# mheinz757/AgglomerationMultigrid1D

Hardware: NVIDIA B200
Metric: FP64 V-cycle DOF-updates/s (higher is better)
Workload: dtype f64

## Files before the change

### agglomerationmultigrid1d_b200/csrc/amg1d.cu

```cuda
#include <cuda_runtime.h>

#include <algorithm>
#include <cmath>
#include <cstdarg>
#include <cstdio>
#include <cstring>
#include <string>
#include <vector>

#ifdef AMG1D_WITH_NCCL
#include <dlfcn.h>
#include <nccl.h>
#endif

#include "../../include/amg1d.h"
#include "kernels_generic.cuh"
#include "kernels_fused.cuh"
#include "kernels_multi.cuh"
#include "kernels_rows.cuh"
#include "direct_bcr.cuh"
#include "device_setup.cuh"
#include "halo_p2p.cuh"

#define AMG1D_VERSION 100
#define PAD_FRONT 64
#define PAD_BACK 64
#define MULTI_SLOTS 8
static_assert(MULTI_MAX_COLS == AMG1D_MAX_COLS, "kernels_multi.cuh and amg1d.h disagree on the column limit");

namespace {

std::string g_create_error;

struct DVec {
    double* raw = nullptr;
    double* p = nullptr;
    int64_t len = 0;
    bool in_arena = false;
};

struct DevBuf {
    double* p = nullptr;
    ~DevBuf() { if (p) cudaFree(p); }
    cudaError_t alloc(int64_t doubles) { return cudaMalloc((void**)&p, (size_t)(doubles > 0 ? doubles : 1) * 8); }
    DevBuf() = default;
    DevBuf(const DevBuf&) = delete;
    DevBuf& operator=(const DevBuf&) = delete;
};

struct Level {
    bool set = false;
    int64_t n = 0;
    int64_t n_glob = 0;
    int64_t start = 0;
    int gl = 0, gr = 0;
    bool sharded = false;
    bool present = true;
    bool proxy = false;
    double* mat_alloc = nullptr;
    int m = 0;
    int diag = 0;
    int K = 0;
    MatDesc md = {};
    int64_t base_n = 0;
    double* flux[9] = {nullptr, nullptr, nullptr, nullptr, nullptr, nullptr, nullptr, nullptr, nullptr};
    bool smooth_tri = false;
    int dv_rec = 0;
    double* smat_alloc = nullptr;
    double* smat = nullptr;
    MatDesc smd = {};
    int64_t n_host = 0;
    double* mat = nullptr;
    int64_t* perm = nullptr;
    std::vector<double> h_lo, h_di, h_up;
    int64_t mat_bytes = 0;
    double* pat = nullptr;
    int pat_head = 0, pat_tail = 0;
    std::vector<double> pat_host;
};

struct Transfer {
    bool set = false;
    int64_t n_fine = 0, n_coarse = 0;
    int mf = 0, mc = 0;
    int64_t* parent = nullptr;
    int64_t* cp = nullptr;
    std::vector<int64_t> h_parent;
    int ratio = 1, shift = 0, base = 0, period = 0, n_head = 0, n_tail = 0;
    double* P0 = nullptr;
    double* P1 = nullptr;
    int64_t nblk = 0;
    bool single_parent_uniform = false;
    bool closed = false;
    bool fusable = false;
    int64_t p_first = 0;
    int reach = 0;
    int64_t cover_extra = 0;
};

struct Column {
    struct Vecs { DVec x[2], b; int cur = 0; };
    std::vector<Vecs> lv;
    double* scal = nullptr;
    double* partial = nullptr;
    struct { DVec x, p, ap; } cg;
};

struct GraphEntry {
    cudaGraphExec_t exec = nullptr;
    int pre = -1, post = -1, norm = -1, zero0 = -1;
    double alpha = 0.0;
    unsigned mask = 0;
    int64_t launches = 0;
    uint64_t stamp = 0;
};

}

struct amg1d {
    int device = 0;
    cudaStream_t stream = nullptr;
    bool own_stream = false;
    int n_levels = 0;
    std::vector<Level> L;
    std::vector<Transfer> T;
    bool finalized = false;
    std::string err;
    DVec scratch;
    double* stage = nullptr;
    int64_t stage_len = 0;
    int64_t partial_cap = 0;
    Column res;
    bool norm_valid = false;
    bool dev_problem = true;
    double* h_scal = nullptr;
    double* coarse_fac = nullptr;
    int opt_fused = 1, opt_graph = 1;
    int64_t opt_coarse_cta = 1024;
    int opt_compress = 1;
    int opt_pdl = 1;
    int opt_rows = 64;
    int opt_rows_rpt = 0;
    int opt_dvrec = 4;
    int opt_dvrec_max = 4;
    int opt_dvreg = 0;
    int opt_pipe = 1;
    int64_t opt_pipe_min = 500000;
    int opt_pattern = 0;
    int tail_start = -1;
    TailLevel* d_tail = nullptr;
    TailPlan tail_plan_ = {};
    std::vector<TailLevel> tail_host;
    uint64_t tail_gen = 0;
    GraphEntry graphs[4];
    uint64_t graph_clock = 0;
    int64_t launches_per_cycle = 0;
    BcrSolver coarse_bcr;
    std::vector<BcrSolver> direct;
    int64_t launch_counter = 0;
    int64_t device_bytes = 0;
    int opt_profile = 0;
    struct Prof { std::vector<cudaEvent_t> ev; };
    std::vector<Prof> prof;
    int rank = 0, nranks = 1;
    int ghost_depth = 4;
    int64_t shard_min = 8192;
    int gather_level = -1;
#ifdef AMG1D_WITH_NCCL
    ncclComm_t comm = nullptr;
#endif
// ... 109 lines not shown
}

int column_alloc(amg1d* h, Column& col, bool cg) {
    const bool levels = col.lv.empty();
    int rc = AMG1D_OK;
    if (levels) {
        col.lv.resize((size_t)h->n_levels);
        for (int l = 0; l < h->n_levels && rc == AMG1D_OK; ++l) {
            const Level& lv = h->L[l];
            Column::Vecs& v = col.lv[(size_t)l];
            if (!lv.present && !lv.proxy) continue;
            const bool arena = lv.sharded && h->p2p.arena;
            for (DVec* d : {&v.x[0], &v.b, &v.x[1]})
                if (rc == AMG1D_OK && (d != &v.x[1] || lv.present))
                    rc = arena ? vec_from_arena(h, *d, lv.n, lv.m) : vec_alloc(h, *d, lv.n, lv.m);
        }
        if (rc == AMG1D_OK) rc = dev_alloc(h, (void**)&col.partial, (h->partial_cap + 256) * 8);
    }
    if (rc == AMG1D_OK && cg && !col.cg.x.raw)
        for (DVec* d : {&col.cg.x, &col.cg.p, &col.cg.ap})
            if (rc == AMG1D_OK) rc = vec_alloc(h, *d, h->L[0].n, h->L[0].m);
    if (rc != AMG1D_OK) {
        if (levels) column_free(h, col);
        else { vec_release(h, col.cg.x); vec_release(h, col.cg.p); vec_release(h, col.cg.ap); }
        cudaGetLastError();
    }
    return rc;
}

inline dim3 gblock(int m) {
    int z = 256 / (AMG1D_TILE * m);
    if (z < 1) z = 1;
    return dim3(AMG1D_TILE, m, z);
}
inline unsigned ggrid(int64_t n, int m) {
    const int z = gblock(m).z;
    return (unsigned)((amg1d_tiles(n) + z - 1) / z);
}

#define LAUNCH_CHECK() CK(cudaGetLastError())

bool valid_level(amg1d* h, int l) { return h && l >= 0 && l < h->n_levels; }

TransferMap make_map(const Transfer& t) {
    TransferMap tm;
    tm.parent = t.parent;
    tm.cp = t.cp;
    tm.n_fine = t.n_fine;
    tm.n_coarse = t.n_coarse;
    tm.ratio = t.ratio;
    tm.shift = t.shift;
    tm.base = t.base;
    tm.period = t.period;
    tm.n_head = t.n_head;
    tm.n_tail = t.n_tail;
    return tm;
}

TransferMap make_map_closed(const Transfer& t) {
    TransferMap tm = make_map(t);
    tm.parent = nullptr;
    tm.cp = nullptr;
    return tm;
}

inline const double* tp0(const Transfer& t) { return t.P0 ? t.P0 - t.p_first * (int64_t)(t.mf * t.mc) : nullptr; }
inline const double* tp1(const Transfer& t) { return t.P1 ? t.P1 - t.p_first * (int64_t)(t.mf * t.mc) : nullptr; }

inline int64_t slab_start(int64_t n_glob, int nranks, int r) { return (n_glob / nranks) * r; }
inline int64_t slab_size(int64_t n_glob, int nranks, int r) {
    return n_glob / nranks + (r == nranks - 1 ? n_glob % nranks : 0);
}

#ifdef AMG1D_WITH_NCCL
struct NcclApi {
    void* lib = nullptr;
    decltype(&ncclGetUniqueId) GetUniqueId = nullptr;
    decltype(&ncclCommInitRank) CommInitRank = nullptr;
    decltype(&ncclCommDestroy) CommDestroy = nullptr;
    decltype(&ncclSend) Send = nullptr;
    decltype(&ncclRecv) Recv = nullptr;
    decltype(&ncclAllReduce) AllReduce = nullptr;
    decltype(&ncclAllGather) AllGather = nullptr;
    decltype(&ncclGroupStart) GroupStart = nullptr;
    decltype(&ncclGroupEnd) GroupEnd = nullptr;
    decltype(&ncclGetErrorString) GetErrorString = nullptr;
};
NcclApi g_nccl;

const char* load_nccl() {
    if (g_nccl.lib) return nullptr;
    const char* env = getenv("AMG1D_NCCL_LIB");
    void* lib = env ? dlopen(env, RTLD_NOW | RTLD_LOCAL) : nullptr;
    if (!lib) lib = dlopen("libnccl.so.2", RTLD_NOW | RTLD_LOCAL);
    if (!lib) lib = dlopen("libnccl.so", RTLD_NOW | RTLD_LOCAL);
    if (!lib) return "cannot dlopen libnccl.so.2";
#define NSYM(field, name)                                                    \
    g_nccl.field = reinterpret_cast<decltype(g_nccl.field)>(dlsym(lib, name)); \
    if (!g_nccl.field) return "libnccl lacks " name;
    NSYM(GetUniqueId, "ncclGetUniqueId") NSYM(CommInitRank, "ncclCommInitRank")
    NSYM(CommDestroy, "ncclCommDestroy") NSYM(Send, "ncclSend") NSYM(Recv, "ncclRecv")
    NSYM(AllReduce, "ncclAllReduce") NSYM(AllGather, "ncclAllGather") NSYM(GroupStart, "ncclGroupStart") NSYM(GroupEnd, "ncclGroupEnd")
    NSYM(GetErrorString, "ncclGetErrorString")
#undef NSYM
    g_nccl.lib = lib;
    return nullptr;
}
#endif

int rows_rpt(const amg1d* h, int l) {
    if (h->opt_rows_rpt) return h->opt_rows_rpt;
    return h->opt_pattern && h->L[l].pat ? 3 : 1;
}

int leg_rec(const amg1d* h, const Level& lv, int mc = 0) {
    int rec = (h->opt_dvrec > 0 && lv.dv_rec && lv.m >= h->opt_dvrec && lv.m <= h->opt_dvrec_max)
                  ? (lv.dv_rec | (h->opt_dvreg ? 8 : 0) | ((h->opt_pipe && lv.n >= h->opt_pipe_min) ? 16 : 0)) : 0;
    if (!rec && h->opt_dvrec > 0 && h->opt_dvreg >= 2 && lv.dv_rec && lv.m == 2 && fused_has_dv(lv.m, mc, lv.md.st, lv.diag))
        rec = lv.dv_rec | 8;
    if (h->opt_dvrec > 0 && h->opt_pipe >= 2 && lv.n >= h->opt_pipe_min && lv.dv_rec && lv.m == 2 &&
        fused_has_pp(lv.m, mc, lv.md.st, lv.diag))
        rec = (rec & 8) | lv.dv_rec | 16;
    return rec;
}

PatOp make_pat(const amg1d* h, int l) {
    const Level& lv = h->L[l];
    PatOp po;
    po.tab = h->opt_pattern ? lv.pat : nullptr;
    po.n_glob = lv.n_glob;
    po.n_head = lv.pat_head;
    po.n_tail = lv.pat_tail;
    po.host_interior = (h->opt_pattern == 2 && lv.pat && !lv.pat_host.empty())
                           ? lv.pat_host.data() + (size_t)lv.pat_head * lv.K : nullptr;
    return po;
}

Slab make_slab(amg1d* h, int l) {
    Slab sl;
    const Level& lv = h->L[l];
    sl.gl = lv.gl;
    sl.gr = lv.gr;
    sl.e_off = lv.start;
    sl.c_off = 0;
    sl.nc = 0;
    if (l + 1 < h->n_levels) {
        const Level& lc = h->L[l + 1];
        sl.c_off = lv.sharded ? slab_start(lc.n_glob, h->nranks, h->rank) : 0;
        sl.nc = lv.sharded ? slab_size(lc.n_glob, h->nranks, h->rank) : lc.n_glob;
    }
    return sl;
}

#ifdef AMG1D_WITH_NCCL
#define NCK(call)                                                                              \
    do {                                                                                       \
        ncclResult_t r_ = (call);                                                              \
        if (r_ != ncclSuccess)                                                                 \
            return fail(h, AMG1D_ERR_NCCL, "%s failed: %s (%s:%d)", #call, g_nccl.GetErrorString(r_), \
                        __FILE__, __LINE__);                                                   \
    } while (0)

int op_halo(amg1d* h, double* v, int64_t n, int m, double* v2 = nullptr, int64_t n2 = 0, int m2 = 0) {
    NCK(g_nccl.GroupStart());
    for (int k = 0; k < 2; ++k) {
        double* p = k == 0 ? v : v2;
        if (!p) continue;
        const int64_t nn = k == 0 ? n : n2;
        const int mm = k == 0 ? m : m2;
        const int64_t cnt = (int64_t)h->ghost_depth * mm;
        if (h->rank > 0) {
            NCK(g_nccl.Send(p, cnt, ncclDouble, h->rank - 1, h->comm, h->stream));
            NCK(g_nccl.Recv(p - cnt, cnt, ncclDouble, h->rank - 1, h->comm, h->stream));
        }
        if (h->rank < h->nranks - 1) {
            NCK(g_nccl.Send(p + (nn - h->ghost_depth) * mm, cnt, ncclDouble, h->rank + 1, h->comm, h->stream));
            NCK(g_nccl.Recv(p + nn * mm, cnt, ncclDouble, h->rank + 1, h->comm, h->stream));
        }
    }
    NCK(g_nccl.GroupEnd());
    h->launch_counter++;
    return AMG1D_OK;
}

int op_gather_rhs(amg1d* h, Column& col, int g) {
    Level& lg = h->L[g];
    double* b = col.lv[(size_t)g].b.p;
    NCK(g_nccl.GroupStart());
    if (h->rank == 0) {
        for (int r = 1; r < h->nranks; ++r)
            NCK(g_nccl.Recv(b + slab_start(lg.n_glob, h->nranks, r) * lg.m,
                            slab_size(lg.n_glob, h->nranks, r) * lg.m, ncclDouble, r, h->comm, h->stream));
    } else {
        NCK(g_nccl.Send(b, slab_size(lg.n_glob, h->nranks, h->rank) * lg.m, ncclDouble, 0, h->comm,
                        h->stream));
    }
    NCK(g_nccl.GroupEnd());
    h->launch_counter++;
    return AMG1D_OK;
}

int op_scatter_sol(amg1d* h, Column& col, int g) {
    Level& lg = h->L[g];
    Column::Vecs& v = col.lv[(size_t)g];
    const int gd = h->ghost_depth;
    NCK(g_nccl.GroupStart());
    if (h->rank == 0) {
        const double* x = v.x[v.cur].p;
        for (int r = 1; r < h->nranks; ++r) {
            const int64_t e0 = slab_start(lg.n_glob, h->nranks, r) - gd;
            const int64_t e1 = slab_start(lg.n_glob, h->nranks, r) + slab_size(lg.n_glob, h->nranks, r) +
                               (r < h->nranks - 1 ? gd : 0);
            NCK(g_nccl.Send(x + e0 * lg.m, (e1 - e0) * lg.m, ncclDouble, r, h->comm, h->stream));
        }
    } else {
        const int64_t cnt = (slab_size(lg.n_glob, h->nranks, h->rank) + gd +
                             (h->rank < h->nranks - 1 ? gd : 0)) * lg.m;
        NCK(g_nccl.Recv(v.x[0].p - (int64_t)gd * lg.m, cnt, ncclDouble, 0, h->comm, h->stream));
    }
    NCK(g_nccl.GroupEnd());
    h->launch_counter++;
    return AMG1D_OK;
}

__global__ void k_sqrt_inplace(double* v, int slot) { v[slot] = sqrt(v[slot]); }
int op_allreduce_max(amg1d* h, double* dptr, int count) {
    NCK(g_nccl.AllReduce(dptr, dptr, (size_t)count, ncclDouble, ncclMax, h->comm, h->stream));
    return AMG1D_OK;
}
int op_allreduce_norm(amg1d* h, Column& col, int slot, bool take_sqrt) {
    NCK(g_nccl.AllReduce(col.scal + slot, col.scal + slot, 1, ncclDouble, ncclSum, h->comm, h->stream));
    h->launch_counter++;
    if (!take_sqrt) return AMG1D_OK;
    k_sqrt_inplace<<<1, 1, 0, h->stream>>>(col.scal, slot);
    h->launch_counter++;
    LAUNCH_CHECK();
    return AMG1D_OK;
}

#define AMG1D_P2P_MAXL 48
struct P2PXchg {
    cudaIpcMemHandle_t hnd;
    int32_t ok, n_sharded;
    int64_t off[AMG1D_P2P_MAXL][3];
    int64_t n[AMG1D_P2P_MAXL];
};

int nccl_allgather_host(amg1d* h, const void* mine, void* all, size_t bytes) {
    DevBuf snd, rcv;
    CK(snd.alloc((int64_t)(bytes + 7) / 8));
    CK(rcv.alloc((int64_t)(bytes * h->nranks + 7) / 8));
    CK(cudaMemcpyAsync(snd.p, mine, bytes, cudaMemcpyHostToDevice, h->stream));
    NCK(g_nccl.AllGather(snd.p, rcv.p, bytes, ncclChar, h->comm, h->stream));
    CK(cudaMemcpyAsync(all, rcv.p, bytes * h->nranks, cudaMemcpyDeviceToHost, h->stream));
    CK(cudaStreamSynchronize(h->stream));
    return AMG1D_OK;
}

int p2p_alloc_arena(amg1d* h) {
    amg1d::P2P& P = h->p2p;
    int n_sh = 0;
    int64_t total = 0;
    for (int l = 0; l < h->n_levels; ++l) {
        const Level& lv = h->L[l];
        if (!lv.sharded) continue;
        ++n_sh;
        total += 3 * arena_round((PAD_FRONT + lv.n * lv.m + PAD_BACK) * 8);
    }
    if (n_sh == 0 || n_sh > AMG1D_P2P_MAXL) return AMG1D_OK;
    P.n_ch = 2 * n_sh;
    const int64_t flag_bytes = arena_round((int64_t)2 * P.n_ch * 8);
    total += flag_bytes;
    if (cudaMalloc((void**)&P.arena, (size_t)total) != cudaSuccess) { cudaGetLastError(); P.arena = nullptr; return AMG1D_OK; }
    CK(cudaMemsetAsync(P.arena, 0, (size_t)total, h->stream));
    h->device_bytes += total;
    P.bytes = total;
    P.used = flag_bytes;
    P.flags = reinterpret_cast<unsigned long long*>(P.arena);
    return AMG1D_OK;
}

void p2p_close(amg1d* h) {
    amg1d::P2P& P = h->p2p;
    for (int s = 0; s < 2; ++s)
        if (P.peer[s]) { cudaIpcCloseMemHandle(P.peer[s]); P.peer[s] = nullptr; }
    P.on = false;
}

int p2p_connect(amg1d* h, Column& col) {
    amg1d::P2P& P = h->p2p;
    if (!P.arena) return AMG1D_OK;
    P2PXchg mine;
    memset(&mine, 0, sizeof mine);
    mine.ok = cudaIpcGetMemHandle(&mine.hnd, P.arena) == cudaSuccess ? 1 : 0;
    if (!mine.ok) cudaGetLastError();
    for (int l = 0; l < h->n_levels && l < AMG1D_P2P_MAXL; ++l) {
        const Level& lv = h->L[l];
        if (!lv.sharded) continue;
        ++mine.n_sharded;
        const Column::Vecs& cv = col.lv[(size_t)l];
        const DVec* v[3] = {&cv.x[0], &cv.x[1], &cv.b};
        for (int k = 0; k < 3; ++k) {
            if (!v[k]->in_arena) mine.ok = 0;
            mine.off[l][k] = reinterpret_cast<const char*>(v[k]->p) - P.arena;
        }
        mine.n[l] = lv.n;
// ... 163 lines not shown
            lv.smat, lv.smd, h->scratch.p, zero_guess ? nullptr : xin, xout, lv.n, alpha);
        h->launch_counter++;
        LAUNCH_CHECK();
        return AMG1D_OK;
    }
    if (h->opt_fused && fused_sweep(lv.md, lv.mat, b, xin, xout, lv.n, alpha, zero_guess, h->stream)) {
        h->launch_counter++;
        LAUNCH_CHECK();
        return AMG1D_OK;
    }
    const dim3 blk = gblock(lv.m);
    const size_t sm = (size_t)blk.z * lv.m * AMG1D_TILE * sizeof(double);
    g_sweep<<<ggrid(lv.n, lv.m), blk, sm, h->stream>>>(lv.mat, lv.md, b, xin, xout, lv.n, alpha,
                                                        zero_guess);
    h->launch_counter++;
    LAUNCH_CHECK();
    return AMG1D_OK;
}

int op_apply(amg1d* h, int l, const double* b, const double* x, double* out, int mode) {
    Level& lv = h->L[l];
    g_apply<<<ggrid(lv.n, lv.m), gblock(lv.m), 0, h->stream>>>(lv.mat, lv.md, b, x, out, lv.n, mode);
    h->launch_counter++;
    LAUNCH_CHECK();
    return AMG1D_OK;
}

int op_restrict(amg1d* h, int l, const double* rf, double* rc) {
    Transfer& t = h->T[l];
    const int64_t total = t.n_coarse * t.mc;
    g_restrict<<<(unsigned)((total + 255) / 256), 256, 0, h->stream>>>(make_map(t), t.mf, t.mc, t.P0,
                                                                       t.P1, rf, rc);
    h->launch_counter++;
    LAUNCH_CHECK();
    return AMG1D_OK;
}

int op_prolong(amg1d* h, int l, const double* xc, double* xf, int add) {
    Transfer& t = h->T[l];
    const int64_t total = t.n_fine * t.mf;
    g_prolong<<<(unsigned)((total + 255) / 256), 256, 0, h->stream>>>(make_map(t), t.mf, t.mc, t.P0,
                                                                      t.P1, xc, xf, add);
    h->launch_counter++;
    LAUNCH_CHECK();
    return AMG1D_OK;
}

int op_coarse(amg1d* h, const double* b, double* x) {
    Level& lv = h->L[h->n_levels - 1];
    if (h->coarse_bcr.ready()) {
        CK(h->coarse_bcr.solve(b, x, h->stream, &h->launch_counter));
        return AMG1D_OK;
    }
    g_coarse_solve<<<1, 32, 2 * lv.m * sizeof(double), h->stream>>>(h->coarse_fac, lv.m, lv.n, b, x);
    h->launch_counter++;
    LAUNCH_CHECK();
    return AMG1D_OK;
}

int op_norm(amg1d* h, Column& col, const double* a, const double* c, int64_t n, int slot) {
    int nb = (int)std::min<int64_t>(AMG1D_RED_BLOCKS, (n + AMG1D_RED_THREADS - 1) / AMG1D_RED_THREADS);
    if (nb < 1) nb = 1;
    k_sqdiff_partial<<<nb, AMG1D_RED_THREADS, 0, h->stream>>>(a, c, n, col.partial);
    k_reduce_final<<<1, AMG1D_RED_THREADS, 0, h->stream>>>(col.partial, nb, col.scal, slot,
                                                           h->nranks > 1 ? 0 : 1);
    h->launch_counter += 2;
    LAUNCH_CHECK();
    if (h->nranks > 1) RET(op_allreduce_norm(h, col, slot, true));
    return AMG1D_OK;
}

int op_reduce_partials(amg1d* h, Column& col, int64_t np, int slot, bool take_sqrt) {
    const double* src = col.partial;
    if (np > 8192) {
        double* stage2 = col.partial + h->partial_cap;
        k_sum_partial<<<256, AMG1D_RED_THREADS, 0, h->stream>>>(col.partial, np, stage2);
        h->launch_counter++;
        src = stage2;
        np = 256;
    }
    k_reduce_final<<<1, AMG1D_RED_THREADS, 0, h->stream>>>(src, (int)np, col.scal, slot,
                                                           take_sqrt && h->nranks == 1 ? 1 : 0);
    h->launch_counter++;
    LAUNCH_CHECK();
    if (h->nranks > 1) RET(op_allreduce_norm(h, col, slot, take_sqrt));
    return AMG1D_OK;
}

int op_resnorm(amg1d* h, Column& col, int l, int slot) {
    Level& lv = h->L[l];
    Column::Vecs& v = col.lv[(size_t)l];
    if (lv.sharded) RET(op_halo(h, v.x[v.cur].p, lv.n, lv.m));
    if (h->opt_fused) {
        int nb = 0;
        if (fused_resnorm(lv.md, lv.mat, v.b.p, v.x[v.cur].p, lv.n, col.partial, h->partial_cap, &nb,
                          h->stream)) {
            h->launch_counter++;
            LAUNCH_CHECK();
            return op_reduce_partials(h, col, nb, slot, true);
        }
    }
    RET(op_apply(h, l, v.b.p, v.x[v.cur].p, h->scratch.p, 1));
    return op_norm(h, col, h->scratch.p, nullptr, lv.n * lv.m, slot);
}

int op_dot(amg1d* h, Column& col, const double* a, const double* c, int64_t n, int slot) {
    int nb = (int)std::min<int64_t>(AMG1D_RED_BLOCKS, (n + AMG1D_RED_THREADS - 1) / AMG1D_RED_THREADS);
    if (nb < 1) nb = 1;
    k_dot_partial<<<nb, AMG1D_RED_THREADS, 0, h->stream>>>(a, c, n, col.partial);
    h->launch_counter++;
    LAUNCH_CHECK();
    return op_reduce_partials(h, col, nb, slot, false);
}

int op_matvec_dot(amg1d* h, Column& col, int l, double* x, double* y, int slot) {
    Level& lv = h->L[l];
    if (lv.sharded) RET(op_halo(h, x, lv.n, lv.m));
    int nb = 0;
    if (h->opt_fused && fused_matvec_dot(lv.md, lv.mat, x, y, lv.n, slot >= 0 ? col.partial : nullptr,
                                         h->partial_cap, &nb, h->stream)) {
        h->launch_counter++;
        LAUNCH_CHECK();
        return slot >= 0 ? op_reduce_partials(h, col, nb, slot, false) : AMG1D_OK;
    }
    RET(op_apply(h, l, nullptr, x, y, 0));
    return slot >= 0 ? op_dot(h, col, x, y, lv.n * lv.m, slot) : AMG1D_OK;
}

int prof_mark(amg1d* h, int level, int leg) {
    if (!h->opt_profile) return AMG1D_OK;
    if (h->prof.size() < (size_t)h->n_levels * 2) h->prof.resize((size_t)h->n_levels * 2);
    cudaEvent_t ev;
    CK(cudaEventCreate(&ev));
    CK(cudaEventRecord(ev, h->stream));
    h->prof[level * 2 + leg].ev.push_back(ev);
    return AMG1D_OK;
}

int leg_down(amg1d* h, Column& col, int l, int nPre, double alpha, bool zero0) {
    Level& lv = h->L[l];
    Transfer& t = h->T[l];
    Level& lc = h->L[l + 1];
    Column::Vecs& v = col.lv[(size_t)l];
    Column::Vecs& vc = col.lv[(size_t)l + 1];
    const bool zero = l > 0 || zero0;
    if (zero) v.cur = 0;
    RET(prof_mark(h, l, 0));
    if (lv.sharded && !zero && !h->p2p.on) RET(op_halo(h, v.x[v.cur].p, lv.n, lv.m));
    if (h->opt_fused && t.fusable && !lv.smooth_tri) {
        const int ob = zero ? 0 : 1 - v.cur;
        cudaError_t le = cudaSuccess;
        const bool p2p = h->p2p.on && lv.sharded;
        const HaloLeg hl = p2p ? make_halo_leg(h, l, true, ob) : HaloLeg();
        int fr = fused_down(lv.md, t.mc, make_map_closed(t), nPre, zero, lv.mat, make_pat(h, l), v.b.p, v.x[v.cur].p,
                            v.x[ob].p, tp0(t), tp1(t), vc.b.p, lv.n, lv.n + (lv.gr ? t.cover_extra : 0),
                            alpha, make_slab(h, l), h->stream, h->opt_pdl != 0, &le, leg_rec(h, lv, t.mc), hl);
        if (fr == FUSED_NA && h->opt_rows) {
            if (p2p) RET(op_p2p_wait_for(h, hl));
            fr = rows_down(lv.md, t.mc, make_map_closed(t), nPre, zero, lv.mat, make_pat(h, l), v.b.p, v.x[v.cur].p,
                           v.x[ob].p, tp0(t), tp1(t), vc.b.p, lv.n, lv.n + (lv.gr ? t.cover_extra : 0), alpha,
                           make_slab(h, l), h->opt_rows, rows_rpt(h, l), h->stream, h->opt_pdl != 0, &le);
            if (fr == FUSED_OK && p2p) {
                if (lc.sharded) RET(op_p2p_push(h, col, 2 * l, l, ob, l + 1, 2));
                else RET(op_p2p_push(h, col, 2 * l, l, ob));
            }
        }
        if (fr == FUSED_ERR) return fail(h, AMG1D_ERR_CUDA, "f_down launch failed on level %d: %s", l, cudaGetErrorString(le));
        if (fr == FUSED_OK) {
            v.cur = ob;
            h->launch_counter++;
            LAUNCH_CHECK();
            RET(prof_mark(h, l, 0));
            return AMG1D_OK;
        }
    }
    if (lv.sharded)
        return fail(h, AMG1D_ERR_UNSUPPORTED, "level %d: sharded levels need the fused kernels "
                    "(a block size / transfer with a fused leg, closed-form transfer, option fused = 1)", l);
    if (zero && nPre == 0) CK(cudaMemsetAsync(v.x[0].p, 0, (size_t)v.x[0].len * 8, h->stream));
    for (int s = 0; s < nPre; ++s) {
        if (zero && s == 0) {
            RET(op_sweep(h, l, v.b.p, v.x[0].p, v.x[0].p, alpha, 1));
        } else {
            RET(op_sweep(h, l, v.b.p, v.x[v.cur].p, v.x[1 - v.cur].p, alpha, 0));
            v.cur = 1 - v.cur;
        }
    }
    if (h->opt_fused && t.single_parent_uniform &&
        fused_residual_restrict(lv.md, t.mc, make_map_closed(t), lv.mat, v.b.p, v.x[v.cur].p, t.P0,
                                vc.b.p, lv.n, h->stream)) {
        h->launch_counter++;
        LAUNCH_CHECK();
    } else {
        RET(op_apply(h, l, v.b.p, v.x[v.cur].p, h->scratch.p, 1));
        RET(op_restrict(h, l, h->scratch.p, vc.b.p));
    }
    return prof_mark(h, l, 0);
}

int leg_up(amg1d* h, Column& col, int l, int nPost, double alpha, bool fuse_norm, bool* norm_done, bool* halo_pushed) {
    *halo_pushed = false;
    Level& lv = h->L[l];
    Transfer& t = h->T[l];
    Column::Vecs& v = col.lv[(size_t)l];
    Column::Vecs& vc = col.lv[(size_t)l + 1];
    RET(prof_mark(h, l, 1));
    if (h->opt_fused && t.fusable && !lv.smooth_tri) {
        int nb = 0;
        cudaError_t le = cudaSuccess;
        const bool p2p = h->p2p.on && lv.sharded;
        const int ob = 1 - v.cur;
        const bool push_inside = l > 0 || ob == 0;
        const HaloLeg hl = p2p ? make_halo_leg(h, l, false, push_inside ? ob : -1) : HaloLeg();
        int fr = fused_up(lv.md, t.mc, make_map_closed(t), nPost, lv.mat, make_pat(h, l), v.b.p, v.x[v.cur].p,
                          v.x[1 - v.cur].p, tp0(t), tp1(t), vc.x[vc.cur].p, lv.n, alpha,
                          fuse_norm ? col.partial : nullptr, h->partial_cap, &nb, make_slab(h, l),
                          h->stream, h->opt_pdl != 0, &le, leg_rec(h, lv, t.mc), hl);
        if (fr == FUSED_OK && p2p && push_inside) *halo_pushed = true;
        if (fr == FUSED_NA && h->opt_rows) {
            if (p2p) RET(op_p2p_wait_for(h, hl));
            fr = rows_up(lv.md, t.mc, make_map_closed(t), nPost, lv.mat, make_pat(h, l), v.b.p, v.x[v.cur].p,
                         v.x[1 - v.cur].p, tp0(t), tp1(t), vc.x[vc.cur].p, lv.n, alpha,
                         fuse_norm ? col.partial : nullptr, h->partial_cap, &nb, make_slab(h, l), h->opt_rows,
                         rows_rpt(h, l), h->stream, h->opt_pdl != 0, &le);
        }
        if (fr == FUSED_ERR) return fail(h, AMG1D_ERR_CUDA, "f_up launch failed on level %d: %s", l, cudaGetErrorString(le));
        if (fr == FUSED_OK) {
            v.cur = 1 - v.cur;
            h->launch_counter++;
            LAUNCH_CHECK();
            RET(prof_mark(h, l, 1));
            if (fuse_norm) {
                RET(op_reduce_partials(h, col, nb, 0, true));
                *norm_done = true;
            }
            return AMG1D_OK;
        }
    }
    if (lv.sharded)
        return fail(h, AMG1D_ERR_UNSUPPORTED, "level %d: sharded levels need the fused kernels", l);
    RET(op_prolong(h, l, vc.x[vc.cur].p, v.x[v.cur].p, 1));
    for (int s = 0; s < nPost; ++s) {
        RET(op_sweep(h, l, v.b.p, v.x[v.cur].p, v.x[1 - v.cur].p, alpha, 0));
        v.cur = 1 - v.cur;
    }
    return prof_mark(h, l, 1);
}

int enqueue_vcycle(amg1d* h, Column& col, int nPre, int nPost, double alpha, bool want_norm, bool zero0) {
    const int nl = h->n_levels;
    const int g = h->gather_level;
    bool norm_done = false;
    if (g >= 0) {
        int need = std::max(nPre, nPost) + 1;
        for (int l = 0; l < nl - 1; ++l)
            if (h->L[l].sharded) need = std::max(need, std::max(nPre, nPost) + 1 + h->T[l].reach);
        if (need > h->ghost_depth)
            return fail(h, AMG1D_ERR_ARG, "nPre / nPost need ghost_depth >= %d (option \"ghost_depth\", "
                        "before the first level is set)", need);
    }
    const int ts = (h->tail_start > 0 && h->L[h->tail_start].present) ? h->tail_start : nl;
    const bool p2p = g >= 0 && h->p2p.on;
    bool u0_pushed = false;
    if (p2p) RET(op_p2p_begin_cycle(h));
    for (int l = 0; l < nl - 1 && l < ts; ++l) {
        Level& lv = h->L[l];
        if (!lv.present) break;
        RET(leg_down(h, col, l, nPre, alpha, zero0));
        if (lv.sharded) {
            Level& lc = h->L[l + 1];
            Column::Vecs& v = col.lv[(size_t)l];
            if (p2p) {
                if (!lc.sharded) RET(op_gather_rhs(h, col, l + 1));
            } else if (lc.sharded) RET(op_halo(h, v.x[v.cur].p, lv.n, lv.m, col.lv[(size_t)l + 1].b.p, lc.n, lc.m));
            else {
                RET(op_halo(h, v.x[v.cur].p, lv.n, lv.m));
                RET(op_gather_rhs(h, col, l + 1));
            }
        }
    }
    if (ts < nl) {
        for (int l = ts; l < nl; ++l) col.lv[(size_t)l].cur = 0;
        cudaError_t te = tail_launch(h->L[ts].m, h->d_tail, nl - ts, h->coarse_fac, nPre, nPost, alpha,
                                     h->tail_plan_, h->stream, h->opt_pdl != 0);
        if (te != cudaSuccess) return fail(h, AMG1D_ERR_CUDA, "f_tail launch failed: %s", cudaGetErrorString(te));
        h->launch_counter++;
    } else if (h->L[nl - 1].present) {
        Column::Vecs& v = col.lv[(size_t)nl - 1];
        if (nl > 1 || zero0) v.cur = 0;
        RET(op_coarse(h, v.b.p, v.x[v.cur].p));
    }
    for (int l = std::min(nl - 2, ts - 1); l >= 0; --l) {
        Level& lv = h->L[l];
        Level& lc = h->L[l + 1];
        Column::Vecs& v = col.lv[(size_t)l];
        if (!lv.present) continue;
        if (lv.sharded && !lc.sharded) RET(op_scatter_sol(h, col, l + 1));
        bool pushed = false;
        RET(leg_up(h, col, l, nPost, alpha, want_norm && l == 0, &norm_done, &pushed));
        if (p2p && lv.sharded) {
            if (l == 0) u0_pushed = pushed;
            else if (!pushed) RET(op_p2p_push(h, col, 2 * l + 1, l, v.cur));
        } else if (lv.sharded && l > 0) RET(op_halo(h, v.x[v.cur].p, lv.n, lv.m));
    }
    Column::Vecs& v0 = col.lv[0];
    if (v0.cur != 0) {
        CK(cudaMemcpyAsync(v0.x[0].p, v0.x[1].p, (size_t)v0.x[0].len * 8, cudaMemcpyDeviceToDevice,
                           h->stream));
        v0.cur = 0;
    }
    if (p2p && h->L[0].sharded && !u0_pushed) RET(op_p2p_push(h, col, 1, 0, 0));
    if (want_norm && !norm_done) RET(op_resnorm(h, col, 0, 0));
    return AMG1D_OK;
}

template <class Enqueue>
int replay_vcycle(amg1d* h, GraphEntry (&cache)[4], const GraphEntry& key, bool parity0, int64_t* launches,
                  Enqueue enqueue) {
    if (!h->opt_graph || h->opt_profile) {
        const int64_t c0 = h->launch_counter;
        RET(enqueue());
        *launches = h->launch_counter - c0;
        return AMG1D_OK;
    }
    GraphEntry* ge = nullptr;
    for (auto& g : cache)
        if (g.exec && g.mask == key.mask && g.pre == key.pre && g.post == key.post && g.alpha == key.alpha &&
            g.norm == key.norm && g.zero0 == key.zero0)
            ge = &g;
    if (!ge) {
        ge = &cache[0];
        for (auto& g : cache) if (!g.exec) { ge = &g; break; } else if (g.stamp < ge->stamp) ge = &g;
        if (ge->exec) { cudaGraphExecDestroy(ge->exec); ge->exec = nullptr; }
        if (!parity0) return fail(h, AMG1D_ERR_STATE, "internal: level-0 buffer parity");
        cudaGraph_t g = nullptr;
        const int64_t c0 = h->launch_counter;
        CK(cudaStreamBeginCapture(h->stream, cudaStreamCaptureModeThreadLocal));
        int rc = enqueue();
        cudaError_t ce = cudaStreamEndCapture(h->stream, &g);
        if (rc != AMG1D_OK) { if (g) cudaGraphDestroy(g); return rc; }
        if (ce != cudaSuccess) return fail(h, AMG1D_ERR_CUDA, "graph capture failed: %s", cudaGetErrorString(ce));
        const int64_t n = h->launch_counter - c0;
        h->launch_counter = c0;
        cudaGraphExec_t exec = nullptr;
        ce = cudaGraphInstantiate(&exec, g, 0);
        cudaGraphDestroy(g);
        if (ce != cudaSuccess) return fail(h, AMG1D_ERR_CUDA, "graph instantiate failed: %s", cudaGetErrorString(ce));
        *ge = key;
        ge->exec = exec;
        ge->launches = n;
    }
    ge->stamp = ++h->graph_clock;
    CK(cudaGraphLaunch(ge->exec, h->stream));
    *launches = ge->launches;
    h->launch_counter += ge->launches;
    return AMG1D_OK;
}

int run_vcycle(amg1d* h, Column& col, int nPre, int nPost, double alpha, bool want_norm, bool zero0 = false) {
    if (nPre < 0 || nPost < 0) return fail(h, AMG1D_ERR_ARG, "nPre and nPost must be >= 0");
    GraphEntry key;
    key.pre = nPre; key.post = nPost; key.alpha = alpha; key.norm = (int)want_norm; key.zero0 = (int)zero0; key.mask = 1;
    RET(replay_vcycle(h, h->graphs, key, col.lv[0].cur == 0, &h->launches_per_cycle,
                      [&] { return enqueue_vcycle(h, col, nPre, nPost, alpha, want_norm, zero0); }));
    h->norm_valid = want_norm;
    return AMG1D_OK;
}
// ... 2076 lines not shown
    if (h->nranks > 1) return fail(h, AMG1D_ERR_UNSUPPORTED, "per-level host operations are single-GPU only");
    if (level < 0 || level >= h->n_levels - 1) return fail(h, AMG1D_ERR_ARG, "transfer %d out of range", level);
    if (!xf || !xc) return fail(h, AMG1D_ERR_ARG, "null vector");
    invalidate_graph(h);
    Column::Vecs& vc = h->res.lv[(size_t)level + 1];
    double* cin = vc.x[1 - vc.cur].p;
    RET(to_device(h, level + 1, xc, cin));
    RET(op_prolong(h, level, cin, h->scratch.p, 0));
    return to_host(h, level, h->scratch.p, xf);
}

int amg1d_coarse_solve(amg1d_t* h, double* x, const double* b) {
    RET(check_ready(h));
    if (h->nranks > 1) return fail(h, AMG1D_ERR_UNSUPPORTED, "per-level host operations are single-GPU only");
    if (!x || !b) return fail(h, AMG1D_ERR_ARG, "null vector");
    invalidate_graph(h);
    const int l = h->n_levels - 1;
    Column::Vecs& v = h->res.lv[(size_t)l];
    double* bin = v.x[1 - v.cur].p;
    RET(to_device(h, l, b, bin));
    RET(op_coarse(h, bin, h->scratch.p));
    return to_host(h, l, h->scratch.p, x);
}

int amg1d_direct_solve(amg1d_t* h, int level, double* x, const double* b) {
    RET(check_ready(h));
    if (h->nranks > 1) return fail(h, AMG1D_ERR_UNSUPPORTED, "per-level host operations are single-GPU only");
    if (!valid_level(h, level)) return fail(h, AMG1D_ERR_ARG, "level %d out of range", level);
    if (!x || !b) return fail(h, AMG1D_ERR_ARG, "null vector");
    if (h->direct.size() < (size_t)h->n_levels) h->direct.resize((size_t)h->n_levels);
    BcrSolver& S = h->direct[(size_t)level];
    if (!S.ready()) RET(bcr_factor(h, S, level));
    invalidate_graph(h);
    Column::Vecs& v = h->res.lv[(size_t)level];
    double* bin = v.x[1 - v.cur].p;
    RET(to_device(h, level, b, bin));
    CK(S.solve(bin, h->scratch.p, h->stream, &h->launch_counter));
    return to_host(h, level, h->scratch.p, x);
}

int amg1d_set_option(amg1d_t* h, const char* key, int64_t value) {
    if (!h || !key) return AMG1D_ERR_ARG;
    invalidate_graph(h);
    if (!strcmp(key, "fused")) h->opt_fused = (int)value;
    else if (!strcmp(key, "graph")) h->opt_graph = (int)value;
    else if (!strcmp(key, "pdl")) h->opt_pdl = (int)value;
    else if (!strcmp(key, "rows_window")) {
        if (value != 0 && !rows_window_ok((int)value)) return fail(h, AMG1D_ERR_ARG, "rows_window must be 0, 32 or 64");
        h->opt_rows = (int)value;
    }
    else if (!strcmp(key, "pattern_resident")) {
        if (value < 0 || value > 2) return fail(h, AMG1D_ERR_ARG, "pattern_resident must be 0, 1 or 2");
        h->opt_pattern = (int)value;
    }
    else if (!strcmp(key, "p2p_halo")) {
        if (h->finalized) return fail(h, AMG1D_ERR_STATE, "'p2p_halo' must be set before amg1d_finalize");
        h->opt_p2p = value != 0;
    }
    else if (!strcmp(key, "dinv_registers")) h->opt_dvreg = (int)value;
    else if (!strcmp(key, "leg_pipeline_min")) {
        if (value < 0) return fail(h, AMG1D_ERR_ARG, "leg_pipeline_min must be >= 0");
        h->opt_pipe_min = value;
    }
    else if (!strcmp(key, "recompute_dinv_max")) {
        if (value < 1 || value > 5) return fail(h, AMG1D_ERR_ARG, "recompute_dinv_max must be in [1, 5]");
        h->opt_dvrec_max = (int)value;
    }
    else if (!strcmp(key, "leg_pipeline")) {
        if (value < 0 || value > 2) return fail(h, AMG1D_ERR_ARG, "leg_pipeline must be 0, 1 or 2");
        h->opt_pipe = (int)value;
    }
    else if (!strcmp(key, "recompute_dinv")) {
        if (value < 0) return fail(h, AMG1D_ERR_ARG, "recompute_dinv must be >= 0");
        h->opt_dvrec = (int)value;
    }
    else if (!strcmp(key, "rows_per_thread")) {
        if (value != 0 && !rows_rpt_ok((int)value)) return fail(h, AMG1D_ERR_ARG, "rows_per_thread must be 0 (auto), 1, 2 or 3");
        h->opt_rows_rpt = (int)value;
    }
    else if (!strcmp(key, "coarse_cta_elems")) {
        h->opt_coarse_cta = value;
        if (h->finalized) { CK(cudaSetDevice(h->device)); CK(cudaStreamSynchronize(h->stream)); RET(build_tail(h)); }
    }
    else if (!strcmp(key, "ghost_depth") || !strcmp(key, "shard_min") || !strcmp(key, "compress")) {
        for (auto& lv : h->L)
            if (lv.set) return fail(h, AMG1D_ERR_STATE, "'%s' must be set before the first level", key);
        if (!strcmp(key, "compress")) { h->opt_compress = value != 0; return AMG1D_OK; }
        if (value < 1) return fail(h, AMG1D_ERR_ARG, "'%s' must be >= 1", key);
        if (!strcmp(key, "ghost_depth")) {
            if ((value + 2) * 8 > PAD_FRONT) return fail(h, AMG1D_ERR_ARG, "ghost_depth must be <= %d", PAD_FRONT / 8 - 2);
            h->ghost_depth = (int)value;
        } else h->shard_min = value;
    }
    else if (!strcmp(key, "profile")) {
        h->opt_profile = (int)value;
        for (auto& pr : h->prof) { for (auto ev : pr.ev) cudaEventDestroy(ev); pr.ev.clear(); }
    }
    else return fail(h, AMG1D_ERR_ARG, "unknown option '%s'", key);
    return AMG1D_OK;
}

int64_t amg1d_get_info(amg1d_t* h, const char* key) {
    if (!h || !key) return -1;
    if (!strcmp(key, "kernel_launches")) return h->launch_counter;
    if (!strcmp(key, "launches_per_cycle")) return h->launches_per_cycle;
    if (!strcmp(key, "device_bytes")) return h->device_bytes;
    if (!strcmp(key, "n_levels")) return h->n_levels;
    if (!strcmp(key, "local_elements")) return h->L[0].n;
    if (!strcmp(key, "local_dofs")) return h->L[0].n * h->L[0].m;
    if (!strcmp(key, "local_offset_dofs")) return h->L[0].start * h->L[0].m;
    if (!strcmp(key, "gather_level")) return h->gather_level;
    if (!strcmp(key, "tail_start")) return h->tail_start;
    if (!strcmp(key, "ghost_depth")) return h->ghost_depth;
    if (!strcmp(key, "rows_window")) return h->opt_rows;
    if (!strcmp(key, "rows_per_thread")) return h->opt_rows_rpt;
    if (!strcmp(key, "pattern_resident")) return h->opt_pattern;
    if (!strncmp(key, "pattern:", 8)) {
        const int l = atoi(key + 8);
        return valid_level(h, l) && h->L[l].pat ? 1 : 0;
    }
    if (!strcmp(key, "recompute_dinv")) return h->opt_dvrec;
    if (!strcmp(key, "dinv_registers")) return h->opt_dvreg;
    if (!strcmp(key, "leg_pipeline")) return h->opt_pipe;
    if (!strcmp(key, "leg_pipeline_min")) return h->opt_pipe_min;
    if (!strncmp(key, "leg_pipeline:", 13)) {
        const int l = atoi(key + 13);
        if (!valid_level(h, l) || !h->L[l].set || l + 1 >= h->n_levels || !h->T[l].fusable) return 0;
        if (h->opt_pattern && h->L[l].pat) return 0;
        const int rec = leg_rec(h, h->L[l], h->T[l].mc);
        return ((rec & 16) && (rec & 3) && fused_has_pp(h->L[l].m, h->T[l].mc, h->L[l].md.st, h->L[l].diag)) ? 1 : 0;
    }
    if (!strcmp(key, "p2p_halo")) return h->p2p.on ? 1 : 0;
    if (!strcmp(key, "halo_bytes_per_cycle")) {
        int64_t bytes = 0;
        const int sides = (h->rank > 0) + (h->rank < h->nranks - 1);
        for (int l = 0; l < h->n_levels; ++l) {
            if (!h->L[l].sharded) continue;
            bytes += 2LL * h->ghost_depth * h->L[l].m * 8 * sides;
            if (l + 1 < h->n_levels && h->L[l + 1].sharded) bytes += (int64_t)h->ghost_depth * h->L[l + 1].m * 8 * sides;
        }
        return bytes;
    }
    if (!strcmp(key, "sharded_levels")) {
        int c = 0;
        for (const auto& lv : h->L) c += lv.sharded ? 1 : 0;
        return c;
    }
    if (!strncmp(key, "dinv_pivots:", 12)) {
        const int l = atoi(key + 12);
        return valid_level(h, l) && h->L[l].set ? (h->L[l].dv_rec == 1) : -1;
    }
    if (!strncmp(key, "dinv_recompute:", 15)) {
        const int l = atoi(key + 15);
        if (!valid_level(h, l) || !h->L[l].set || l + 1 >= h->n_levels || !(leg_rec(h, h->L[l], h->T[l].mc) & 3)) return 0;
        if (h->opt_pattern && h->L[l].pat) return 0;
        return (h->L[l].m <= 5 && h->T[l].fusable) ? 1 : 0;
    }
    if (!strncmp(key, "structure:", 10)) {
        const int l = atoi(key + 10);
        return valid_level(h, l) && h->L[l].set ? h->L[l].md.st : -1;
    }
    if (!strncmp(key, "tile_rows:", 10)) {
        const int l = atoi(key + 10);
        return valid_level(h, l) && h->L[l].set ? h->L[l].md.K : -1;
    }
    if (!strcmp(key, "rank")) return h->rank;
    if (!strcmp(key, "nranks")) return h->nranks;
    if (!strcmp(key, "dof_updates_per_sweep")) {
        int64_t s = 0;
        for (int l = 0; l < h->n_levels - 1; ++l) s += h->L[l].n_glob * h->L[l].m;
        return s;
    }
    if (!strcmp(key, "multi_columns")) return h->multi.k;
    if (!strcmp(key, "multi_launches_per_cycle")) return h->multi.launches_per_cycle;
    if (!strcmp(key, "multi_pcg_launches_per_iteration")) return h->multi.pcg_launches;
    if (!strncmp(key, "multi_legs:", 11)) {
        const int l = atoi(key + 11);
        if (!valid_level(h, l) || !h->finalized || h->nranks > 1 || l + 1 >= h->n_levels) return 0;
        if (h->tail_start > 0 && l >= h->tail_start) return 0;
        return multi_leg_level(h, l) ? 1 : 0;
    }
    return -1;
}

int amg1d_get_profile(amg1d_t* h, int level, int leg, double* total_ms, int* launches) {
    if (!h || !total_ms || !launches) return AMG1D_ERR_ARG;
    if (!valid_level(h, level) || leg < 0 || leg > 1) return fail(h, AMG1D_ERR_ARG, "bad level / leg");
    *total_ms = 0.0;
    *launches = 0;
    if (h->prof.size() <= (size_t)(level * 2 + leg)) return AMG1D_OK;
    CK(cudaStreamSynchronize(h->stream));
    auto& ev = h->prof[level * 2 + leg].ev;
    for (size_t i = 0; i + 1 < ev.size(); i += 2) {
        float ms = 0.f;
        CK(cudaEventElapsedTime(&ms, ev[i], ev[i + 1]));
        *total_ms += ms;
        *launches += 1;
    }
    return AMG1D_OK;
}

int amg1d_host_alloc(void** p, int64_t bytes) {
    amg1d* h = nullptr;
    if (!p || bytes < 0) return fail(h, AMG1D_ERR_ARG, "bad arguments");
    CK(cudaMallocHost(p, (size_t)std::max<int64_t>(bytes, 8)));
    return AMG1D_OK;
}

int amg1d_host_free(void* p) {
    amg1d* h = nullptr;
    if (p) CK(cudaFreeHost(p));
    return AMG1D_OK;
}

}
```

Baseline: 232.1 billion.

## Add two-elements-per-thread fused down/up leg kernels for m=2 coarse levels

Adds new fused smoothing+restriction and prolongation+smoothing kernels in which each thread owns two adjacent elements, exchanging neighbours through double-buffered shared memory and loading matrix tiles as double2. The kernels recompute diagonal inverses in registers and are used on non-sharded intermediate levels with m=2, eligible structures and transfer ratios 1 or 2. The aim is to halve shared-memory exchange traffic and thread count per element and to vectorize loads, cutting per-leg cost on mid levels. It adds a new code path gated by several conditions and falls back to the existing fused kernels otherwise.

```diff
diff --git a/agglomerationmultigrid1d_b200/csrc/amg1d.cu b/agglomerationmultigrid1d_b200/csrc/amg1d.cu
--- a/agglomerationmultigrid1d_b200/csrc/amg1d.cu
+++ b/agglomerationmultigrid1d_b200/csrc/amg1d.cu
@@ -16,6 +16,7 @@
 #include "../../include/amg1d.h"
 #include "kernels_generic.cuh"
 #include "kernels_fused.cuh"
+#include "kernels_pair.cuh"
 #include "kernels_multi.cuh"
 #include "kernels_rows.cuh"
 #include "direct_bcr.cuh"
@@ -431,6 +432,15 @@
     return sl;
 }
 
+bool pair_legs(amg1d* h, int l) {
+    if (l < 1 || l + 1 >= h->n_levels || (h->tail_start > 0 && l >= h->tail_start)) return false;
+    const Level& lv = h->L[l];
+    const Transfer& t = h->T[l];
+    return h->opt_fused && h->opt_dvrec > 0 && lv.set && lv.dv_rec && !lv.sharded && !(h->opt_pattern && lv.pat) &&
+           t.fusable && !lv.smooth_tri && leg_rec(h, lv, t.mc) == 0 &&
+           pair_legs_ok(lv.md, t.mc, make_map_closed(t), t.P1 != nullptr, make_slab(h, l));
+}
+
 #ifdef AMG1D_WITH_NCCL
 #define NCK(call)                                                                              \
     do {                                                                                       \
@@ -900,7 +910,12 @@
         cudaError_t le = cudaSuccess;
         const bool p2p = h->p2p.on && lv.sharded;
         const HaloLeg hl = p2p ? make_halo_leg(h, l, true, ob) : HaloLeg();
-        int fr = fused_down(lv.md, t.mc, make_map_closed(t), nPre, zero, lv.mat, make_pat(h, l), v.b.p, v.x[v.cur].p,
+        int fr = pair_legs(h, l) ? pair_down(lv.md, t.mc, make_map_closed(t), nPre, zero, lv.mat, v.b.p, v.x[ob].p,
+                                             tp0(t), tp1(t), vc.b.p, lv.n, alpha, make_slab(h, l), h->stream,
+                                             h->opt_pdl != 0, &le, lv.dv_rec)
+                                 : FUSED_NA;
+        if (fr == FUSED_NA)
+            fr = fused_down(lv.md, t.mc, make_map_closed(t), nPre, zero, lv.mat, make_pat(h, l), v.b.p, v.x[v.cur].p,
                             v.x[ob].p, tp0(t), tp1(t), vc.b.p, lv.n, lv.n + (lv.gr ? t.cover_extra : 0),
                             alpha, make_slab(h, l), h->stream, h->opt_pdl != 0, &le, leg_rec(h, lv, t.mc), hl);
         if (fr == FUSED_NA && h->opt_rows) {
@@ -960,7 +975,13 @@
         const int ob = 1 - v.cur;
         const bool push_inside = l > 0 || ob == 0;
         const HaloLeg hl = p2p ? make_halo_leg(h, l, false, push_inside ? ob : -1) : HaloLeg();
-        int fr = fused_up(lv.md, t.mc, make_map_closed(t), nPost, lv.mat, make_pat(h, l), v.b.p, v.x[v.cur].p,
+        int fr = pair_legs(h, l) ? pair_up(lv.md, t.mc, make_map_closed(t), nPost, lv.mat, v.b.p, v.x[v.cur].p,
+                                           v.x[1 - v.cur].p, tp0(t), tp1(t), vc.x[vc.cur].p, lv.n, alpha,
+                                           fuse_norm ? col.partial : nullptr, make_slab(h, l), h->stream,
+                                           h->opt_pdl != 0, &le, lv.dv_rec)
+                                 : FUSED_NA;
+        if (fr == FUSED_NA)
+            fr = fused_up(lv.md, t.mc, make_map_closed(t), nPost, lv.mat, make_pat(h, l), v.b.p, v.x[v.cur].p,
                           v.x[1 - v.cur].p, tp0(t), tp1(t), vc.x[vc.cur].p, lv.n, alpha,
                           fuse_norm ? col.partial : nullptr, h->partial_cap, &nb, make_slab(h, l),
                           h->stream, h->opt_pdl != 0, &le, leg_rec(h, lv, t.mc), hl);
@@ -3343,9 +3364,14 @@
     }
     if (!strncmp(key, "dinv_recompute:", 15)) {
         const int l = atoi(key + 15);
+        if (valid_level(h, l) && pair_legs(h, l)) return 1;
         if (!valid_level(h, l) || !h->L[l].set || l + 1 >= h->n_levels || !(leg_rec(h, h->L[l], h->T[l].mc) & 3)) return 0;
         if (h->opt_pattern && h->L[l].pat) return 0;
         return (h->L[l].m <= 5 && h->T[l].fusable) ? 1 : 0;
+    }
+    if (!strncmp(key, "leg_pairs:", 10)) {
+        const int l = atoi(key + 10);
+        return valid_level(h, l) && pair_legs(h, l) ? 1 : 0;
     }
     if (!strncmp(key, "structure:", 10)) {
         const int l = atoi(key + 10);
diff --git a/agglomerationmultigrid1d_b200/csrc/kernels_pair.cuh b/agglomerationmultigrid1d_b200/csrc/kernels_pair.cuh
--- /dev/null
+++ b/agglomerationmultigrid1d_b200/csrc/kernels_pair.cuh
@@ -0,0 +1,281 @@
+#pragma once
+#include "kernels_fused.cuh"
+
+#ifndef PAIR_B
+#define PAIR_B 128
+#endif
+#ifndef PAIR_MINB
+#define PAIR_MINB 4
+#endif
+
+template <int B>
+struct PairExchange {
+    double lf[2][2][B + 2];
+    double rt[2][2][B + 2];
+};
+
+template <int B>
+__device__ __forceinline__ void pair_exch_init(PairExchange<B>& ex) {
+    const int t = threadIdx.x;
+    if (t < 16) {
+        const int buf = t >> 3, i = (t >> 2) & 1, slot = (t & 1) ? B + 1 : 0;
+        if (t & 2) ex.rt[buf][i][slot] = 0.0; else ex.lf[buf][i][slot] = 0.0;
+    }
+}
+
+template <int B, int ST>
+__device__ __forceinline__ void pair_exchange(PairExchange<B>& ex, int buf, int ilo, const double (&x0)[2],
+                                              const double (&x1)[2], double (&nl)[2], double (&nr)[2]) {
+    const int t = threadIdx.x;
+    ex.lf[buf][0][t + 1] = x0[0];
+    ex.lf[buf][1][t + 1] = x0[1];
+    if constexpr (ST == AMG1D_ST_COLROW) {
+        ex.rt[buf][0][t + 1] = ilo ? x1[1] : x1[0];
+    } else {
+        ex.rt[buf][0][t + 1] = x1[0];
+        ex.rt[buf][1][t + 1] = x1[1];
+    }
+    __syncthreads();
+    if constexpr (ST == AMG1D_ST_COLROW) {
+        nl[0] = ex.rt[buf][0][t];
+        nl[1] = 0.0;
+    } else {
+        nl[0] = ex.rt[buf][0][t];
+        nl[1] = ex.rt[buf][1][t];
+    }
+    nr[0] = ex.lf[buf][0][t + 2];
+    nr[1] = ex.lf[buf][1][t + 2];
+}
+
+template <int ST>
+__device__ __forceinline__ void pair_left_of_1(int ilo, const double (&x0)[2], double (&xl)[2]) {
+    if constexpr (ST == AMG1D_ST_COLROW) { xl[0] = ilo ? x0[1] : x0[0]; xl[1] = 0.0; }
+    else { xl[0] = x0[0]; xl[1] = x0[1]; }
+}
+
+template <int ST>
+__device__ __forceinline__ void pair_sweep(const RegOpDv<2, ST>& A0, const RegOpDv<2, ST>& A1, int ilo, int iup,
+                                           const double (&b0)[2], const double (&b1)[2], const double (&nl)[2],
+                                           double (&x0)[2], double (&x1)[2], const double (&nr)[2], double alpha,
+                                           bool zg) {
+    double l1[2];
+    pair_left_of_1<ST>(ilo, x0, l1);
+    const double r0[2] = {x1[0], x1[1]};
+    reg_sweep<2, ST, false, 1>(A0, ilo, iup, nullptr, b0, nl, x0, r0, alpha, zg);
+    reg_sweep<2, ST, false, 1>(A1, ilo, iup, nullptr, b1, l1, x1, nr, alpha, zg);
+}
+
+template <int ST>
+__device__ __forceinline__ void pair_load(const double* __restrict__ mat, int64_t e, bool a0, bool a1, int rec,
+                                          RegOpDv<2, ST>& A0, RegOpDv<2, ST>& A1) {
+    using S = OpShape<2, ST>;
+    constexpr int K = S::O_DV + 4;
+    const double* T = mat + (e >> 5) * (int64_t)(K * AMG1D_TILE) + (e & 31);
+    if (a1) {
+#pragma unroll
+        for (int k = 0; k < S::NO; ++k) {
+            const double2 v = *reinterpret_cast<const double2*>(T + k * AMG1D_TILE);
+            A0.lo[k] = v.x; A1.lo[k] = v.y;
+        }
+#pragma unroll
+        for (int k = 0; k < 4; ++k) {
+            const double2 v = *reinterpret_cast<const double2*>(T + (S::O_DI + k) * AMG1D_TILE);
+            A0.di[k] = v.x; A1.di[k] = v.y;
+        }
+#pragma unroll
+        for (int k = 0; k < S::NO; ++k) {
+            const double2 v = *reinterpret_cast<const double2*>(T + (S::O_UP + k) * AMG1D_TILE);
+            A0.up[k] = v.x; A1.up[k] = v.y;
+        }
+    } else {
+#pragma unroll
+        for (int k = 0; k < S::NO; ++k) { A0.lo[k] = a0 ? T[k * AMG1D_TILE] : 0.0; A1.lo[k] = 0.0; }
+#pragma unroll
+        for (int k = 0; k < 4; ++k) { A0.di[k] = a0 ? T[(S::O_DI + k) * AMG1D_TILE] : 0.0; A1.di[k] = 0.0; }
+#pragma unroll
+        for (int k = 0; k < S::NO; ++k) { A0.up[k] = a0 ? T[(S::O_UP + k) * AMG1D_TILE] : 0.0; A1.up[k] = 0.0; }
+    }
+#pragma unroll
+    for (int k = 0; k < 4; ++k) { A0.dv[k] = A0.di[k]; A1.dv[k] = A1.di[k]; }
+    const bool piv = (rec & 3) != 2;
+    if (a0) { if (piv) reg_invert<2, true>(A0.dv); else reg_invert<2, false>(A0.dv); }
+    if (a1) { if (piv) reg_invert<2, true>(A1.dv); else reg_invert<2, false>(A1.dv); }
+}
+
+__device__ __forceinline__ void pair_load_vec(const double* __restrict__ p, int64_t e, bool a0, bool a1,
+                                              double (&v0)[2], double (&v1)[2]) {
+    if (a0) load_vec<2>(p + e * 2, v0); else { v0[0] = 0.0; v0[1] = 0.0; }
+    if (a1) load_vec<2>(p + e * 2 + 2, v1); else { v1[0] = 0.0; v1[1] = 0.0; }
+}
+
+__device__ __forceinline__ void pair_store_vec(double* __restrict__ p, int64_t e, bool a0, bool a1,
+                                               const double (&v0)[2], const double (&v1)[2]) {
+    if (a0) store_vec<2>(p + e * 2, v0);
+    if (a1) store_vec<2>(p + e * 2 + 2, v1);
+}
+
+__device__ __forceinline__ void pair_restrict_add(const double* __restrict__ P0, const TransferMap& tm, const WinIdx& wi,
+                                                  int64_t c, int tc, const double (&r)[2], double (&acc)[2]) {
+    const double* P = P0 + win_blk(tm, wi, c, tc) * 4;
+#pragma unroll
+    for (int j = 0; j < 2; ++j)
+#pragma unroll
+        for (int i = 0; i < 2; ++i) acc[j] = fma(P[j * 2 + i], r[i], acc[j]);
+}
+
+__device__ __forceinline__ void pair_correct(const double* __restrict__ P0, const TransferMap& tm, const WinIdx& wi,
+                                             int64_t c, int tc, const double* __restrict__ c0, double (&x)[2]) {
+    const int64_t pb = win_blk(tm, wi, c, tc) * 4;
+    double y[2] = {0.0, 0.0};
+#pragma unroll
+    for (int j = 0; j < 2; ++j) {
+        const double cj = c0[j];
+#pragma unroll
+        for (int i = 0; i < 2; ++i) y[i] = fma(P0[pb + j * 2 + i], cj, y[i]);
+    }
+#pragma unroll
+    for (int i = 0; i < 2; ++i) x[i] = x[i] + y[i];
+}
+
+template <int ST, int RATIO, int NSW>
+__global__ void __launch_bounds__(PAIR_B, PAIR_MINB)
+f_down_pair(const double* __restrict__ mat, int ilo, int iup, const double* __restrict__ b, double* __restrict__ xout,
+            const double* __restrict__ P0, TransferMap tm, double* __restrict__ rc, int64_t n, double alpha, int nsweep,
+            WinIdx wi, int rec) {
+    __shared__ PairExchange<PAIR_B> ex;
+    pdl_launch_dependents();
+    const int t = threadIdx.x;
+    const int64_t e = (int64_t)blockIdx.x * wi.out - wi.halo + 2 * t;
+    const bool a0 = e >= 0 && e < n, a1 = e >= 0 && e + 1 < n;
+    pair_exch_init<PAIR_B>(ex);
+    RegOpDv<2, ST> A0, A1;
+    pair_load<ST>(mat, e, a0, a1, rec, A0, A1);
+    pdl_wait();
+    double b0[2], b1[2];
+    pair_load_vec(b, e, a0, a1, b0, b1);
+    double x0[2] = {0.0, 0.0}, x1[2] = {0.0, 0.0}, nl[2], nr[2];
+    __syncthreads();
+    int buf = 0;
+    const int ns = NSW > 0 ? NSW : nsweep;
+#pragma unroll
+    for (int s = 0; s < ns; ++s) {
+        if (s > 0) {
+            pair_exchange<PAIR_B, ST>(ex, buf, ilo, x0, x1, nl, nr);
+            buf ^= 1;
+        }
+        pair_sweep<ST>(A0, A1, ilo, iup, b0, b1, nl, x0, x1, nr, alpha, s == 0);
+    }
+    const bool mine = 2 * t >= wi.halo && 2 * t < wi.halo + wi.out;
+    if (mine) pair_store_vec(xout, e, a0, a1, x0, x1);
+    pair_exchange<PAIR_B, ST>(ex, buf, ilo, x0, x1, nl, nr);
+    double r0[2], r1[2];
+    {
+        double l1[2];
+        pair_left_of_1<ST>(ilo, x0, l1);
+        reg_residual<2, ST>(A0, ilo, iup, b0, nl, x0, x1, r0);
+        reg_residual<2, ST>(A1, ilo, iup, b1, l1, x1, nr, r1);
+    }
+    if (!mine || !a0 || e >= tm.n_fine) return;
+    if constexpr (RATIO == 2) {
+        const int64_t Kc = (int64_t)blockIdx.x * wi.opr + wi.qdiv0 + t + tm.base;
+        if (Kc >= 0 && Kc < tm.n_coarse) {
+            double acc[2] = {0.0, 0.0};
+            pair_restrict_add(P0, tm, wi, e, 2 * t, r0, acc);
+            if (e + 1 < tm.n_fine) pair_restrict_add(P0, tm, wi, e + 1, 2 * t + 1, r1, acc);
+            store_vec<2>(rc + Kc * 2, acc);
+        }
+    } else {
+        const int64_t Kc = (int64_t)blockIdx.x * wi.opr + wi.qdiv0 + 2 * t + tm.base;
+#pragma unroll
+        for (int k = 0; k < 2; ++k) {
+            if (e + k < tm.n_fine && Kc + k >= 0 && Kc + k < tm.n_coarse) {
+                double acc[2] = {0.0, 0.0};
+                pair_restrict_add(P0, tm, wi, e + k, 2 * t + k, k ? r1 : r0, acc);
+                store_vec<2>(rc + (Kc + k) * 2, acc);
+            }
+        }
+    }
+}
+
+template <int ST, int RATIO, int NSW>
+__global__ void __launch_bounds__(PAIR_B, PAIR_MINB)
+f_up_pair(const double* __restrict__ mat, int ilo, int iup, const double* __restrict__ b,
+          const double* __restrict__ xin, double* __restrict__ xout, const double* __restrict__ P0, TransferMap tm,
+          const double* __restrict__ xcoarse, int64_t n, double alpha, int nsweep, WinIdx wi, int rec) {
+    __shared__ PairExchange<PAIR_B> ex;
+    pdl_launch_dependents();
+    const int t = threadIdx.x;
+    const int64_t e = (int64_t)blockIdx.x * wi.out - wi.halo + 2 * t;
+    const bool a0 = e >= 0 && e < n, a1 = e >= 0 && e + 1 < n;
+    pair_exch_init<PAIR_B>(ex);
+    RegOpDv<2, ST> A0, A1;
+    pair_load<ST>(mat, e, a0, a1, rec, A0, A1);
+    pdl_wait();
+    double b0[2], b1[2], x0[2], x1[2], nl[2], nr[2];
+    pair_load_vec(b, e, a0, a1, b0, b1);
+    pair_load_vec(xin, e, a0, a1, x0, x1);
+    const int64_t par = (int64_t)blockIdx.x * wi.opr + wi.qdiv0 + (RATIO == 2 ? t : 2 * t) + tm.base;
+    if (a0) pair_correct(P0, tm, wi, e, 2 * t, xcoarse + par * 2, x0);
+    if (a1) pair_correct(P0, tm, wi, e + 1, 2 * t + 1, xcoarse + (RATIO == 2 ? par : par + 1) * 2, x1);
+    __syncthreads();
+    int buf = 0;
+    const int ns = NSW > 0 ? NSW : nsweep;
+#pragma unroll
+    for (int s = 0; s < ns; ++s) {
+        pair_exchange<PAIR_B, ST>(ex, buf, ilo, x0, x1, nl, nr);
+        buf ^= 1;
+        pair_sweep<ST>(A0, A1, ilo, iup, b0, b1, nl, x0, x1, nr, alpha, false);
+    }
+    if (2 * t >= wi.halo && 2 * t < wi.halo + wi.out) pair_store_vec(xout, e, a0, a1, x0, x1);
+}
+
+inline bool pair_legs_ok(const MatDesc& d, int mc, const TransferMap& tm, bool two_parent, const Slab& sl) {
+    const bool st_ok = d.st == AMG1D_ST_DENSE || (d.st == AMG1D_ST_COLROW && d.iup == FUSED_COLROW_IUP);
+    const bool map_ok = tm.ratio == 1 || (tm.ratio == 2 && tm.shift % 2 == 0);
+    return d.m == 2 && mc == 2 && !d.diag && st_ok && !two_parent && map_ok && sl.gl == 0 && sl.gr == 0 &&
+           sl.e_off == 0 && sl.c_off == 0;
+}
+
+inline WinIdx pair_window(int nsweep, const TransferMap& tm, const Slab& sl) {
+    return fused_window(nsweep | 1, tm, false, sl, 2 * PAIR_B);
+}
+
+inline int pair_down(const MatDesc& d, int mc, const TransferMap& tm, int nsweep, bool zero, const double* mat,
+                     const double* b, double* xout, const double* P0, const double* P1, double* rc, int64_t n,
+                     double alpha, const Slab& sl, cudaStream_t st, bool pdl, cudaError_t* err, int rec) {
+    if (!zero || !pair_legs_ok(d, mc, tm, P1 != nullptr, sl) || ((uintptr_t)mat | (uintptr_t)b | (uintptr_t)xout) & 15)
+        return FUSED_NA;
+    const WinIdx w = pair_window(nsweep, tm, sl);
+    if (w.out < 2 || w.qmod0 != 0) return FUSED_NA;
+    const unsigned grid = (unsigned)((n + w.out - 1) / w.out);
+#define PD(SS, RR)                                                                                                \
+    if (d.st == SS && tm.ratio == RR) {                                                                           \
+        *err = launch_fused(nsweep == 3 ? f_down_pair<SS, RR, 3> : f_down_pair<SS, RR, 0>, grid, PAIR_B, 0, st, pdl, \
+                            mat, d.ilo, d.iup, b, xout, P0, tm, rc, n, alpha, nsweep, w, rec);                    \
+        return *err == cudaSuccess ? FUSED_OK : FUSED_ERR;                                                        \
+    }
+    PD(AMG1D_ST_COLROW, 2) PD(AMG1D_ST_DENSE, 2) PD(AMG1D_ST_COLROW, 1) PD(AMG1D_ST_DENSE, 1)
+#undef PD
+    return FUSED_NA;
+}
+
+inline int pair_up(const MatDesc& d, int mc, const TransferMap& tm, int nsweep, const double* mat, const double* b,
+                   const double* xin, double* xout, const double* P0, const double* P1, const double* xcoarse,
+                   int64_t n, double alpha, const double* partial, const Slab& sl, cudaStream_t st, bool pdl,
+                   cudaError_t* err, int rec) {
+    if (partial || !pair_legs_ok(d, mc, tm, P1 != nullptr, sl) ||
+        ((uintptr_t)mat | (uintptr_t)b | (uintptr_t)xin | (uintptr_t)xout) & 15)
+        return FUSED_NA;
+    const WinIdx w = pair_window(nsweep, tm, sl);
+    if (w.out < 2 || w.qmod0 != 0) return FUSED_NA;
+    const unsigned grid = (unsigned)((n + w.out - 1) / w.out);
+#define PU(SS, RR)                                                                                                \
+    if (d.st == SS && tm.ratio == RR) {                                                                           \
+        *err = launch_fused(nsweep == 3 ? f_up_pair<SS, RR, 3> : f_up_pair<SS, RR, 0>, grid, PAIR_B, 0, st, pdl,   \
+                            mat, d.ilo, d.iup, b, xin, xout, P0, tm, xcoarse, n, alpha, nsweep, w, rec);          \
+        return *err == cudaSuccess ? FUSED_OK : FUSED_ERR;                                                        \
+    }
+    PU(AMG1D_ST_COLROW, 2) PU(AMG1D_ST_DENSE, 2) PU(AMG1D_ST_COLROW, 1) PU(AMG1D_ST_DENSE, 1)
+#undef PU
+    return FUSED_NA;
+}
```

Measured after the change: 244.2 billion, median of 6. +5.2%, better.
